# alp-aydin/Raytracing-Project

Measured on AMD Instinct MI355X. Metric: Mrays/s (primary+secondary) + wall-clock per frame, 4K scene @1/2/4/8 GPU, higher is better.
Workload: dtype f64; 1 GPU; snorlax 3840x2160, 5 lights, rec 4 (config 4); width=3840, height=2160, mode=standard, rays_per_frame=385232714, rays_traced_per_frame=385232714, parallelism=1 ranks, 1 GPU each: row-strips8x1, cull=True

## Files before the change

raytracing-project_amd/csrc/device/rt_device.hpp:

```cpp
#include <hip/hip_runtime.h>
#include <stdint.h>

#include <type_traits>

#include "rt.h"
#include "rt_launch.hpp"
#include "scene_compile.hpp"

#ifndef RT_REAL
#define RT_REAL double
#define RT_NS rtd
#endif

namespace RT_NS {

using rtamd::DevObj;
using rtamd::DevOp;
using real = RT_REAL;
using NodeT = rtamd::NodeR<real>;
using MatT = rtamd::MatR<real>;
using LightT = rtamd::LightR<real>;
using DLightT = rtamd::DLightR<real>;
using FoldT = rtamd::FoldLeafR<real>;
#define RT_STR2(x) #x
// ... 52 lines not shown
    const double rcp = __builtin_amdgcn_rcp(s0);
    const double f0 = __builtin_fma(-s0, rcp, 1.0);
    const double f1 = __builtin_fma(rcp, f0, rcp);
    const double f2 = __builtin_fma(-s0, f1, 1.0);
    const double f3 = __builtin_fma(f1, f2, f1);
    auto quot = [&](double a) {
        bool vcc;
        const double n = __builtin_amdgcn_div_scale(a, b, true, &vcc);
        const double mul = n * f3;
        const double f4 = __builtin_fma(-s0, mul, n);
        return __builtin_amdgcn_div_fixup(__builtin_amdgcn_div_fmas(f4, f3, mul, vcc), b, a);
    };
    return D3{quot(a0), quot(a1), quot(a2)};
}
__device__ __forceinline__ auto div3(float a0, float a1, float a2, float b) {
    struct F3 { float x, y, z; };
    return F3{a0 / b, a1 / b, a2 / b};
}

#ifndef RT_FUSED_NORM
#define RT_FUSED_NORM 1
#endif
static_assert(!RT_FUSED_NORM || std::is_same_v<real, double>, "RT_FUSED_NORM is FP64 only (rt_kernels_f32.hip sets it to 0)");

__device__ __forceinline__ double sqrt_core(double s, double& h) {
    const double y = __builtin_amdgcn_rsq(s);
    double g = s * y;
    h = y * 0.5;
    const double r = __builtin_fma(-h, g, 0.5);
    g = __builtin_fma(g, r, g);
    h = __builtin_fma(h, r, h);
    const double d0 = __builtin_fma(-g, g, s);
    g = __builtin_fma(d0, h, g);
    const double d1 = __builtin_fma(-g, g, s);
    return __builtin_fma(d1, h, g);
}

__device__ __forceinline__ D3 div3(double a0, double a1, double a2, double L, double h) {
    const double y0 = h + h;
    const double e = __builtin_fma(-L, y0, 1.0);
    const double y = __builtin_fma(y0, e, y0);
    auto quot = [&](double a) {
        const double q = a * y;
        const double r = __builtin_fma(-L, q, a);
        return __builtin_fma(r, y, q);
    };
// ... 82 lines not shown
    PH_CHAIN_XF,
    PH_OBJ_PREF,
    PH_OBJ_HIT,
    PH_WAVE_SETUP,
    PH_COUNT
};
enum RtEvent {
    EV_SHQ = 0,
    EV_SH_CAND,
    EV_SH_HIT,
    EV_SH_CSG,
    EV_PR_CAND,
    EV_PR_HIT,
    EV_FOLD_LEAF,
    EV_COMB,
    EV_COMB_SINGLE,
    EV_COMB_EASY,
    EV_COMB_GEN,
    EV_LIGHT1,
    EV_LIGHT2,
    EV_BOUNCE,
    EV_COMPACT_LEAF,
    EV_WAVES,
    EV_COUNT
};
template <bool C>
struct Cnt;
template <>
struct Cnt<false> {
    static constexpr bool kPlain = false;
    __device__ __forceinline__ void inc(int) {}
    __device__ __forceinline__ void gate(bool) {}
#ifdef RT_EVENT_PROF
    __device__ static unsigned long long* acc() {
        __shared__ unsigned long long a[4][EV_COUNT];
        return &a[threadIdx.x >> 6][0];
    }
    __device__ __forceinline__ void init() {
        if ((threadIdx.x & 63) == 0)
            for (int k = 0; k < EV_COUNT; ++k) acc()[k] = 0;
    }
    __device__ __forceinline__ bool first() {
        return (int)__lane_id() == __builtin_ctzll(__builtin_amdgcn_read_exec());
    }
    __device__ __forceinline__ void ev(int k) {
        if (first()) acc()[k] += 1;
    }
// ... 579 lines not shown
        real t1 = (-half_b + s) / RV(1.0);
        if (t0 > t1) {
            const real tt = t0;
            t0 = t1;
            t1 = tt;
        }
        o.t0 = t0;
        o.t1 = t1;
        if (o.ok) cnt.inc(RT_OPC_SPHERE_IVL_HIT);
    }
    o.s0 = o.t0;
    o.s1 = o.t1;
}

template <class CT>
__device__ __forceinline__ void csg_c(int op, const CIvl& A, const CIvl& B, CIvl& R, CT& cnt) {
    R.ok = 0;
    R.t0 = R.t1 = R.s0 = R.s1 = RV(0.0);
    R.c0 = R.c1 = 0;
    if (!A.ok && !B.ok) return;
    cnt.inc(RT_OPC_CSG_COMBINE);
    cnt.ev(EV_COMB);
    if (!(A.ok && B.ok)) {
        cnt.ev(EV_COMB_SINGLE);
        const bool useA = A.ok;
        if (op == RT_CSG_INTERSECTION || (op == RT_CSG_DIFFERENCE && !useA)) return;
        const CIvl& X = useA ? A : B;
        const bool inX = (X.t0 < RV(1e-6)) && (X.t1 > RV(1e-6));
        R.t1 = X.t1;
        R.s1 = X.s1;
        R.c1 = X.c1;
        if (inX) {
            R.ok = __builtin_isfinite(X.t1);
            R.t0 = RV(0.0);
            R.s0 = X.s0;
            R.c0 = (X.c0 & ~REF_FLIP) | REF_ORIGIN;
        } else {
            R.ok = __builtin_isfinite(X.t0) && __builtin_isfinite(X.t1) && !ev_less(X.t1, 1, X.t0, 0);
            R.t0 = X.t0;
            R.s0 = X.s0;
            R.c0 = X.c0;
        }
        return;
    }
    if (op == RT_CSG_UNION) {
        const real e = RV(1e-6);
        const bool easy = __builtin_isfinite(A.t0) && __builtin_isfinite(A.t1) && __builtin_isfinite(B.t0) &&
                          __builtin_isfinite(B.t1) && (A.t1 - A.t0 > e) && (B.t1 - B.t0 > e) &&
                          (fabs_r(A.t0 - B.t0) > e) && (fabs_r(A.t0 - B.t1) > e) && (fabs_r(A.t1 - B.t0) > e) &&
                          (fabs_r(A.t1 - B.t1) > e);
        if (easy) {
            cnt.ev(EV_COMB_EASY);
            const bool inA = (A.t0 < e) && (A.t1 > e);
            const bool inB = (B.t0 < e) && (B.t1 > e);
            const bool xa = inA || (!inB && A.t0 < B.t0);
            const real x1 = xa ? A.t1 : B.t1;
            const real y0 = xa ? B.t0 : A.t0;
            const real y1 = xa ? B.t1 : A.t1;
            const bool ext_y = (y0 < x1) && (y1 > x1);
            const bool org = inA || inB;
            const int xc0 = xa ? A.c0 : B.c0;
            R.ok = 1;
            R.t0 = org ? RV(0.0) : (xa ? A.t0 : B.t0);
            R.s0 = xa ? A.s0 : B.s0;
            R.c0 = org ? ((xc0 & ~REF_FLIP) | REF_ORIGIN) : xc0;
            R.t1 = ext_y ? y1 : x1;
            R.s1 = (ext_y != xa) ? A.s1 : B.s1;
            R.c1 = (ext_y != xa) ? A.c1 : B.c1;
            return;
        }
    }
    cnt.ev(EV_COMB_GEN);
    real et[4];
    int ec[4];
#pragma unroll
    for (int k = 0; k < 4; ++k) {
        et[k] = RV(0.0);
        ec[k] = 0;
    }
    int n = 0;
    {
        const real tv[4] = {A.t0, A.t1, B.t0, B.t1};
        const bool pv[4] = {A.ok && __builtin_isfinite(A.t0), A.ok && __builtin_isfinite(A.t1),
                            B.ok && __builtin_isfinite(B.t0), B.ok && __builtin_isfinite(B.t1)};
#pragma unroll
        for (int e = 0; e < 4; ++e) {
#pragma unroll
            for (int k = 0; k < 4; ++k) {
                const bool here = pv[e] && n == k;
                et[k] = here ? tv[e] : et[k];
                ec[k] = here ? e : ec[k];
            }
            n += pv[e] ? 1 : 0;
        }
    }
// ... 560 lines not shown
    const f2v qxy = pk_fma(f2s(-s), K.uxy, wxy);
    const float qz = __builtin_fmaf(-s, K.uz, wz);
    const float d2 = dot_pk(qxy, qz, qxy, qz);
    const float R = g.w + K.rho + __builtin_fmaf(1e-5f, gmag, K.m5);
    return !(d2 > R * R);
}
__device__ __forceinline__ bool capsule_touch(const float* g, const Capsule& K) {
    const float4 b = *reinterpret_cast<const float4*>(g);
    return capsule_touch(b, ball_mag(b), K);
}


__device__ __forceinline__ bool record_touch(const float4 c0, const float4 c1, const Capsule& K) {
    const int type = __float_as_int(c1.x);
    const f2v sab = pk_fma(f2s(c0.x), K.abx, pk_fma(f2s(c0.y), K.aby, f2s(c0.z) * K.abz)) - f2s(c0.w);
    const float m = __builtin_fmaf(1e-5f, c1.y, K.rm5);
    const bool plane = !((sab.x > m) & (sab.y > m)) & !((sab.x < -m) & (sab.y < -m));
    const bool ball = capsule_touch(c0, c1.y, K);
    return (type == 1) | ((type == 2) & ball) | ((type == 3) & plane);
}

template <bool EAGER, bool DEEP, bool UO, bool BV = false, bool LEAD = false, class CT>
__device__ bool scene_occluded_capsule(const DevScene& S, const DRay& r0, real tmin, real tmax, bool need, bool wave_ok,
                                    CT& cnt, bool regular = true) {
#if defined(RT_ABL) && RT_ABL == 1
    return false;
#endif
    cnt.pb(PH_WAVE_SETUP);
    const FRay fr = to_fray(r0);
    DRay r = r0;
    bool r_exact = false;
    const float ftmin = (float)tmin, ftmax = (float)tmax;
    const uint64_t nm = __ballot(need);
    if (!nm) return false;
    cnt.ev(EV_SHQ);
    const int f = __builtin_ctzll(nm);
    const float Ax = __builtin_fmaf(ftmin, fr.dx, fr.ox), Ay = __builtin_fmaf(ftmin, fr.dy, fr.oy),
                Az = __builtin_fmaf(ftmin, fr.dz, fr.oz);
    const float Bx = __builtin_fmaf(ftmax, fr.dx, fr.ox), By = __builtin_fmaf(ftmax, fr.dy, fr.oy),
                Bz = __builtin_fmaf(ftmax, fr.dz, fr.oz);
    const bool fin = __builtin_isfinite(Ax + Ay + Az + Bx + By + Bz) && regular;
    const bool cap = wave_ok && exec_full() && !__any(need && !fin);
    const float ax = rdlane_f(Ax, f), ay = rdlane_f(Ay, f), az = rdlane_f(Az, f);
    const float bx = rdlane_f(Bx, f), by = rdlane_f(By, f), bz = rdlane_f(Bz, f);
    const float da = (Ax - ax) * (Ax - ax) + (Ay - ay) * (Ay - ay) + (Az - az) * (Az - az);
    const float db = (Bx - bx) * (Bx - bx) + (By - by) * (By - by) + (Bz - bz) * (Bz - bz);
    const float d = need ? __builtin_fmaxf(da, db) : 0.0f;
// ... 52 lines not shown
        const int nc = S.n_objs - base;
        const int j = base + lane;
        const int jr = j < S.n_objs ? j : S.n_objs - 1;
        const float4 c0 = S.ctab[2 * jr], c1 = S.ctab[2 * jr + 1];
        const bool pass = (j < S.n_objs) &
                          (cap ? record_touch(c0, c1, K)
                               : __float_as_int(c1.x) != 0);
        m = (cap && exec_full()) ? __ballot(pass) : (nc >= 64 ? ~0ull : ((1ull << nc) - 1));
        cnt.pe(PH_WAVE_SETUP);
#if defined(RT_ABL) && RT_ABL == 2
        if (m != 12345) return false;
#endif
        if constexpr (kCounting<CT>) {
            if (need) {
                int skipped = 0;
                for (int o = base; o < S.n_objs && o < base + 64; ++o) {
                    const int k = S.objs[o].kind;
                    if (k != rtamd::OBJ_GROUP && k != rtamd::OBJ_NEVER && !((m >> (o - base)) & 1)) ++skipped;
                }
                cnt_add(cnt, RT_OPC_CULLED, skipped);
            }
        }
        }
        while (m) {
            const int o = base + __builtin_ctzll(m);
            m &= m - 1;
            const DevObj ob = S.objs[o];
            if (ob.kind == rtamd::OBJ_GROUP || ob.kind == rtamd::OBJ_NEVER) continue;
            cnt.ev(EV_SH_CAND);
            cnt.pb(PH_OBJ_PREF);
            uint64_t lmask = ~0ull;
            bool use_mask = false;
            if (kCsg<CT> && cap && ob.npb > 0 && exec_full()) {
                const float* g = S.gb + 4 * (ob.pb0 + (lane < ob.npb ? lane : 0));
                const bool in = lane < ob.npb;
                const uint64_t cb = __ballot(in && capsule_touch(g, K));
                bool seg = cb != 0;
#ifndef RT_NO_LANE_LEAF_TEST
                if (seg) {
                    seg = false;
                    for (uint64_t mm = cb; mm && !seg; mm &= mm - 1) {
                        const float* gk = S.gb + 4 * (ob.pb0 + __builtin_ctzll(mm));
                        seg = __any(need && !hit && ball_touch(gk, fr, ftmin, ftmax));
                    }
                }
#endif
                if (!seg) {
                    if (need) cnt.inc(RT_OPC_CULLED);
                    cnt.pe(PH_OBJ_PREF);
                    continue;
                }
                if (!lb_ready) {
                    lb_ready = true;
// ... 396 lines not shown
            }
            cnt.pe(PH_OBJ_HIT);
            if (csg_obj) cnt.pe(PH_SHADOW_CSG);
            if (__all(hit || !need)) return hit;
        }
    }
    return hit;
}


__device__ __forceinline__ bool cone_touch(const float4 g, float gmag, const Cone& K) {
    return cone_touch_t<false>(g, gmag, K);
}
__device__ __forceinline__ bool cone_touch(const float* g, const Cone& K) {
    const float4 b = *reinterpret_cast<const float4*>(g);
    return cone_touch_t<false>(b, ball_mag(b), K);
}

#ifndef RT_CAM_RHO0
#define RT_CAM_RHO0 1
#endif
template <bool EAGER, bool DEEP, bool BV = false, bool LEAD = false, bool CAM = false, class CT>
__device__ bool scene_intersect_wave(const DevScene& S, const DRay& r, real tmin, real tmax, real& t_best,
                                     DHit& best, bool wave_ok, CT& cnt, bool valid = true) {
    cnt.pb(PH_WAVE_SETUP);
    const uint64_t vm = __ballot(valid);
    if (!vm) {
        cnt.pe(PH_WAVE_SETUP);
        return false;
    }
    const int f = __builtin_ctzll(vm);
    const FRay fr = to_fray(r);
    const bool fin = __builtin_isfinite(fr.ox + fr.oy + fr.oz + fr.dx + fr.dy + fr.dz);
    const bool cone = S.cull && wave_ok && exec_full() && !__any(valid && !fin) && tmin >= RV(0.0);
    const float ox = rdlane_f(fr.ox, f), oy = rdlane_f(fr.oy, f), oz = rdlane_f(fr.oz, f);
    const float ax = rdlane_f(fr.dx, f), ay = rdlane_f(fr.dy, f), az = rdlane_f(fr.dz, f);
    const float dc = valid ? __builtin_fmaxf(0.0f, 1.0f - __builtin_fmaf(fr.dx, ax, __builtin_fmaf(fr.dy, ay, fr.dz * az)))
                           : 0.0f;
    float rho = 0.0f;
    if constexpr (!(CAM && RT_CAM_RHO0)) {
        const float do2 = valid ? (fr.ox - ox) * (fr.ox - ox) + (fr.oy - oy) * (fr.oy - oy) + (fr.oz - oz) * (fr.oz - oz)
                                : 0.0f;
        rho = cone ? sqrt_cull(__uint_as_float(wave_max_u32(__float_as_uint(do2)))) : 0.0f;
    }
    const float dcm = cone ? __uint_as_float(wave_max_u32(__float_as_uint(dc))) + 4e-6f : 2.0f;
    const float cth = 1.0f - dcm;
    const bool wide = !(cth > 0.0f);
    const float sth = sqrt_cull(__builtin_fmaxf(0.0f, 1.0f - cth * cth)) + 1e-6f;
// ... 109 lines not shown
                                         (t == closest && (win < 0 ? tie : (oo > win_orig ? tie : !win_tie))));
                if (take) {
                    closest = t;
                    win = o;
                    win_orig = oo;
                    win_tie = tie;
                    wp = p;
                    wts = ts;
                    wcode = code;
                }
            } else if (object_hit<EAGER, DEEP>(S, ob, r, tmin, closest, t, p, ts, code, cnt, lmask, use_mask)) {
                closest = t;
                win = o;
                wp = p;
                wts = ts;
                wcode = code;
            }
            cnt.gate(true);
            cnt.pe(PH_OBJ_HIT);
            if (csg_obj) cnt.pe(PH_PRIMARY_CSG);
        }
    }
    if (win < 0) return false;
    cnt.gate(valid);
    resolve_hit<EAGER>(S, win, r, tmin, wp, wts, wcode, best, cnt);
    cnt.gate(true);
    t_best = closest;
    return true;
}

__device__ __attribute__((noinline)) double pow_general(double x, double y) { return pow(x, y); }
#ifndef RT_POW_ANY_X
#define RT_POW_ANY_X 0
#endif

__device__ __forceinline__ double pow_spec(double x, double y) {
    const int k = (int)y;
    if (!(y >= 0.0 && y < 1024.0 && (double)k == y && (!RT_POW_ANY_X || __builtin_fabs(x) <= 2.0)))
        return pow_general(x, y);
    if (k == 0) return 1.0;
    const int top = 31 - __builtin_clz(k);
    double h = x, l = 0.0;
    for (int i = top - 1; i >= 0; --i) {
        double p = h * h;
        l = __builtin_fma(h + h, l, __builtin_fma(h, h, -p));
        h = p;
// ... 8 lines not shown
__device__ __forceinline__ float pow_spec(float x, float y) { return pow(x, y); }

#ifndef RT_LIGHT_CACHE
#define RT_LIGHT_CACHE 5
#endif
constexpr int kLightCache = RT_LIGHT_CACHE;
constexpr int kPoolWave = (kLightCache > 0 ? kLightCache : 1) * 4 * 64;
constexpr size_t pool_bytes(int threads) { return (size_t)(threads / 64) * kPoolWave * sizeof(double); }
__device__ __forceinline__ double* lds_pool() {
    extern __shared__ double rt_lds_pool[];
    return rt_lds_pool;
}
__device__ __forceinline__ double* wave_pool(int w) { return lds_pool() + (size_t)w * kPoolWave; }

__device__ __forceinline__ V3 combine(V3 a, V3 b) {
    return v3(RV(1.0) - (RV(1.0) - a.x) * (RV(1.0) - b.x), RV(1.0) - (RV(1.0) - a.y) * (RV(1.0) - b.y), RV(1.0) - (RV(1.0) - a.z) * (RV(1.0) - b.z));
}

#ifndef RT_STD_UO
#define RT_STD_UO false
#endif
template <bool EAGER, bool DEEP, bool DL, int WV, bool UO = RT_STD_UO, bool LEAD = false, class CT>
__device__ V3 shade(const DevScene& S, real ht, const DHit& hit, V3 wo, uint32_t& n_occl, CT& cnt,
                    bool valid = true) {
    const bool has_mat = hit.mat >= 0;
    valid = valid && has_mat;
    if (valid) cnt.inc(RT_OPC_SHADE_CALL);
    const bool wave_full = WV && __builtin_amdgcn_read_exec() == ~0ull;
    const V3 n = hit.n;
    const real eps = cmax(RV(1e-3), RV(1e-4) * ht);
    ShadowHull hull{0.0f, 0.0f, 0.0f, 0.0f, 0.0f, false};
    if constexpr (WV == 2) hull = shadow_hull<UO>(hit.p, eps, valid, wave_full);
    V3 E = v3(RV(0.0), RV(0.0), RV(0.0));
    {
        const MatT* m = &S.mats[valid ? hit.mat : 0];
        E = v3(m->ambient[0], m->ambient[1], m->ambient[2]);
    }
    for (int li = 0; DL && li < S.n_dlights; ++li) {
        if (!valid) break;
        const DLightT* L = &S.dlights[li];
        cnt.inc(RT_OPC_LIGHT_EVAL);
        const V3 wi = normalized(v3(-L->dir[0], -L->dir[1], -L->dir[2]));
        const real ndotl = dmax(RV(0.0), dot3(n, wi));
        if (ndotl <= RV(0.0)) continue;
        const V3 so = v3(hit.p.x + n.x * eps, hit.p.y + n.y * eps, hit.p.z + n.z * eps);
        ++n_occl;
        if (scene_occluded<EAGER, DEEP>(S, make_ray(so, wi), eps, RT_INF, cnt)) continue;
        cnt.inc(RT_OPC_SHADE_LIGHT);
        const MatT* m = &S.mats[hit.mat];
        const real sd = m->kd * ndotl;
        const V3 Ed = v3(m->albedo[0] * L->radiance[0] * sd, m->albedo[1] * L->radiance[1] * sd,
                         m->albedo[2] * L->radiance[2] * sd);
        V3 Es = v3(RV(0.0), RV(0.0), RV(0.0));
        if (m->ks > RV(0.0)) {
            cnt.inc(RT_OPC_SHADE_SPEC);
            const V3 rr = normalized(v3(RV(2.0) * dot3(n, wi) * n.x - wi.x, RV(2.0) * dot3(n, wi) * n.y - wi.y,
                                        RV(2.0) * dot3(n, wi) * n.z - wi.z));
            const real rdotv = dmax(RV(0.0), dot3(rr, wo));
            const real spec = pow_spec(rdotv, m->shininess) * m->ks;
            Es = v3(L->radiance[0] * spec, L->radiance[1] * spec, L->radiance[2] * spec);
        }
        E = combine(E, combine(Ed, Es));
    }
    if (WV) cnt.pb(PH_SHADE2);
    double* const lc = wave_pool((int)(threadIdx.x >> 6)) + (threadIdx.x & 63);
    for (int l0 = 0; __any(valid) && l0 < S.n_lights; l0 += 32) {
        const int l1 = S.n_lights - l0 < 32 ? S.n_lights : l0 + 32;
        uint32_t lit = 0;
        if (WV) cnt.pb(PH_SHADE1);
        for (int li = l0; li < l1; ++li) {
            const LightT* L = &S.lights[li];
            if (valid) cnt.inc(RT_OPC_LIGHT_EVAL);
            V3 tl = v3(L->pos[0] - hit.p.x, L->pos[1] - hit.p.y, L->pos[2] - hit.p.z);
            real d2 = dot3(tl, tl);
            const bool clamped = d2 <= RV(0.01);
            if (clamped) d2 = RV(0.01);
#if RT_FUSED_NORM
            const N3 dw = sqrt_div3(tl.x, tl.y, tl.z, d2, valid);
            const real dist = dw.L;
            const auto wq = dw.q;
#else
            const real dist = sqrt_r(d2);
            const auto wq = div3(tl.x, tl.y, tl.z, dist);
#endif
            const V3 wi = v3(wq.x, wq.y, wq.z);
            if (li - l0 < kLightCache) {
                double* c = lc + (li - l0) * 4 * 64;
                c[0] = wi.x;
                c[64] = wi.y;
                c[2 * 64] = wi.z;
                c[3 * 64] = dist;
            }
            const real ndotl = cmax(RV(0.0), dot3(n, wi));
            const real max_t = dist - eps;
            const bool need = valid && ndotl > RV(0.0) && max_t > eps;
            if (!__any(need)) continue;
            cnt.ev(EV_LIGHT1);
            const V3 so = v3(hit.p.x + n.x * eps, hit.p.y + n.y * eps, hit.p.z + n.z * eps);
            bool occ = false;
            if constexpr (WV == 2) {
                cnt.pb(PH_SHADOW);
                occ = scene_occluded_wave<EAGER, DEEP, UO, true>(S, DRay{so, wi}, eps, max_t, need, wave_full, cnt, li,
                                                                 hull, !clamped);
                cnt.pe(PH_SHADOW);
            } else if constexpr (WV) {
                cnt.pb(PH_SHADOW);
                occ = scene_occluded_capsule<EAGER, DEEP, UO, false, LEAD>(S, DRay{so, wi}, eps, max_t, need, wave_full, cnt,
                                                                           !clamped);
                cnt.pe(PH_SHADOW);
            } else if (need) {
                occ = scene_occluded<EAGER, DEEP>(S, DRay{so, wi}, eps, max_t, cnt, true, !clamped);
            }
            if (need) {
                ++n_occl;
                if (!occ) lit |= 1u << (li - l0);
            }
        }
        if (WV) {
            cnt.pe(PH_SHADE1);
            cnt.pb(PH_SHADE2);
        }
#if defined(RT_ABL) && RT_ABL == 4
        if (lit != 12345u) continue;
#endif
        if (!lit) continue;
        const MatT* m = &S.mats[hit.mat];
        const real kd = m->kd, ks = m->ks, shin = m->shininess;
        const V3 alb = ld3(m->albedo);
        for (int li = l0; li < l1; ++li) {
            if (!((lit >> (li - l0)) & 1u)) continue;
            cnt.ev(EV_LIGHT2);
// ... 79 lines not shown
    bool alive = true;
    const bool wave_ok = __builtin_amdgcn_read_exec() == ~0ull;
    auto step = [&](auto first_tag) __attribute__((always_inline)) {
        constexpr bool FIRST = decltype(first_tag)::value;
        const bool eval = alive && depth < limit;
        DRay r;
        if constexpr (FIRST) {
            r = r0;
        } else {
            r = DRay{v3(RV(0.0), RV(0.0), RV(0.0)), v3(RV(0.0), RV(0.0), -RV(1.0))};
            if (eval) r = nxt[rsel];
        }
        if (!FIRST) {
            cnt.ev(EV_BOUNCE);
            cnt.evn(EV_COMPACT_LEAF, (unsigned)__builtin_popcountll(__ballot(eval)));
        }
        real ht = RV(0.0);
        DHit h;
        h.p = h.n = v3(RV(0.0), RV(0.0), RV(0.0));
        h.mat = -1;
        h.ff = 1;
        if (eval) ++n_isect;
        cnt.pb(PH_PRIMARY);
        const bool hit = scene_intersect_wave<EAGER, DEEP, (WV == 2), kCsg<CT> ? RT_SEC_LEAD_I : RT_PLAIN_SEC_LEAD>(S, r, RV(1e-4), RT_INF, ht, h, wave_ok, cnt, eval);
        cnt.pe(PH_PRIMARY);
        const bool sh = eval && hit;
        bool descend = false;
        if (sh && h.mat >= 0) {
            const MatT* mat = &S.mats[h.mat];
            const bool can = depth < limit - 1;
            const bool want_refl = mat->kr > RV(0.0) && can;
            bool want_refr = false;
            DRay refr;
            if (mat->kt > RV(0.0) && can) {
                const real eta = h.ff ? (S.medium_index / mat->refractive_index)
                                      : (mat->refractive_index / S.medium_index);
                const V3 inc = normalized(r.d);
                const real cos_i = -dot3(inc, h.n);
                const real st2 = eta * eta * dmax(RV(0.0), RV(1.0) - cos_i * cos_i);
                if (!(st2 >= RV(1.0))) {
                    want_refr = true;
                    const real cos_t = sqrt_r(RV(1.0) - st2);
                    const real k = eta * cos_i - cos_t;
                    const V3 rd = normalized(v3(inc.x * eta + h.n.x * k, inc.y * eta + h.n.y * k,
                                                inc.z * eta + h.n.z * k));
                    const V3 ro = h.ff ? v3(h.p.x - h.n.x * RV(1e-6), h.p.y - h.n.y * RV(1e-6), h.p.z - h.n.z * RV(1e-6))
                                       : v3(h.p.x + h.n.x * RV(1e-6), h.p.y + h.n.y * RV(1e-6), h.p.z + h.n.z * RV(1e-6));
// ... 2 lines not shown
            }
            if (want_refl || want_refr) {
                WFrame& fr = stk[sp];
                fr.mat = h.mat;
                if (want_refr) nxt[2 * sp + 1] = refr;
                cnt.inc(RT_OPC_SECONDARY);
                if (want_refl) {
                    const V3 inc = normalized(r.d);
                    const real k = RV(2.0) * dot3(inc, h.n);
                    const V3 rd = normalized(v3(inc.x - h.n.x * k, inc.y - h.n.y * k, inc.z - h.n.z * k));
                    const V3 ro = h.ff ? v3(h.p.x + h.n.x * RV(1e-6), h.p.y + h.n.y * RV(1e-6), h.p.z + h.n.z * RV(1e-6))
                                       : v3(h.p.x - h.n.x * RV(1e-6), h.p.y - h.n.y * RV(1e-6), h.p.z - h.n.z * RV(1e-6));
                    fr.sf = want_refr ? 2 : 0;
                    nxt[2 * sp] = make_ray(ro, rd);
                } else {
                    fr.sf = 1;
                }
                ++sp;
                descend = true;
            }
        }
        const V3 wo = normalized(vneg(r.d));
        V3 direct = v3(RV(0.0), RV(0.0), RV(0.0));
        if (__any(sh)) direct = shade<EAGER, DEEP, DL, WV, RT_STD_UO, kCsg<CT> ? RT_SEC_LEAD_S : RT_PLAIN_SEC_LEAD>(S, ht, h, wo, n_occl, cnt, sh);
        V3 ret = v3(RV(0.0), RV(0.0), RV(0.0));
        if (eval && !hit) ret = background(S);
        if (sh) {
            if (descend) {
                stk[sp - 1].total = direct;
                rsel = 2 * (sp - 1) + (stk[sp - 1].sf & 1);
                depth = sp;
            } else {
                ret = direct;
            }
        }
        if (alive && !descend) {
            bool resumed = false;
            while (sp > 0) {
                WFrame& fr = stk[sp - 1];
                const MatT* mat = &S.mats[fr.mat];
                const int sf = fr.sf;
                if ((sf & 1) == 0) {
                    fr.total = combine(fr.total, v3(ret.x * mat->kr, ret.y * mat->kr, ret.z * mat->kr));
                    if (sf & 2) {
                        cnt.inc(RT_OPC_SECONDARY);
                        fr.sf = sf | 1;
                        rsel = 2 * (sp - 1) + 1;
// ... 15 lines not shown
            }
        }
        return ret;
    };
    const V3 first = step(std::true_type{});
    if (!__any(alive)) return first;
    while (__any(alive)) step(std::false_type{});
    return stk[0].total;
}

template <bool EAGER, bool DEEP, bool SECONDARY, bool DL, int WV, class CT>
__device__ __forceinline__ V3 trace(const DevScene& S, DRay r, uint32_t& n_isect, uint32_t& n_occl, CT& cnt) {
#ifndef RT_OLD_TRACE
    if constexpr (SECONDARY && WV) return trace_wave<EAGER, DEEP, DL, WV>(S, r, n_isect, n_occl, cnt);
#endif
    if constexpr (!SECONDARY) {
        if (S.rec_limit <= 0) return v3(RV(0.0), RV(0.0), RV(0.0));
        real ht = RV(0.0);
        DHit h;
        h.mat = -1;
        ++n_isect;
        if constexpr (WV) {
            cnt.pb(PH_PRIMARY);
            const bool hit = scene_intersect_wave<EAGER, DEEP, (WV == 2), false, true>(S, r, RV(1e-4), RT_INF, ht, h,
                                                               __builtin_amdgcn_read_exec() == ~0ull, cnt);
            cnt.pe(PH_PRIMARY);
            if (!__any(hit)) return background(S);
#if defined(RT_ABL) && RT_ABL == 5
            if (S.n_objs != 12345) return hit ? h.n : background(S);
#endif
            const V3 E = shade<EAGER, DEEP, DL, WV>(S, ht, h, normalized(vneg(r.d)), n_occl, cnt, hit);
            return hit ? E : background(S);
        } else {
            if (!scene_intersect<EAGER, DEEP>(S, r, RV(1e-4), RT_INF, ht, h, cnt)) return background(S);
            return shade<EAGER, DEEP, DL, WV>(S, ht, h, normalized(vneg(r.d)), n_occl, cnt);
        }
    }
    Frame stk[kMaxDepth];
    int sp = 0;
    int depth = 0;
    const int limit = S.rec_limit;
    V3 ret;
    for (;;) {
        bool descend = false;
        if (depth >= limit) {
            ret = v3(RV(0.0), RV(0.0), RV(0.0));
        } else {
            real ht = RV(0.0);
            DHit h;
            ++n_isect;
            if (!scene_intersect<EAGER, DEEP>(S, r, RV(1e-4), RT_INF, ht, h, cnt)) {
                ret = background(S);
            } else {
                const V3 wo = normalized(vneg(r.d));
// ... 141 lines not shown
```

raytracing-project_amd/csrc/device/rt_kernels.hpp:

```cpp

namespace RT_NS {

using rtamd::kCounterSlots;
using rtamd::kCounterWords;
using rtamd::PaperParams;
using rtamd::SceneView;
using rtamd::StdParams;

namespace {

#ifndef RT_STD_WPB
#define RT_STD_WPB 1
#endif
constexpr int kStdWPB = RT_STD_WPB;
constexpr int kStdThreads = 64 * kStdWPB;
#ifndef RT_STD_TW
#define RT_STD_TW 2
#endif
constexpr int kStdTW = RT_STD_TW, kStdTH = 8 / RT_STD_TW;
static_assert(kStdTW * kStdTH == 8, "a wave holds 8 pixels");
constexpr int kStdBlockX = kStdWPB >= 2 ? 2 * kStdTW : kStdTW;
constexpr int kStdBlockY = kStdWPB >= 4 ? 2 * kStdTH : kStdTH;

template <bool C, int NWAVES = 4>
// ... 189 lines not shown
#ifndef RT_PAPER_LEAD_S
#define RT_PAPER_LEAD_S true
#endif
template <bool E, bool D, bool C, bool DL = true, int WV = 0, bool T = false, bool PL = false>
__device__ __forceinline__ void paper_primary_body(const DevScene& S, const PaperParams& P) {
    static_assert(!(PL && C), "plain kernels do not count");
    const int lane = threadIdx.x & 63;
    const int x = paper_tile_x() * 8 + (lane & 7);
    const int li = paper_tile_y() * 8 + (lane >> 3);
    const int ei = li < P.n_list ? P.ext_list[li] : -1;
    const bool active = x < P.W && ei >= 0;
    unsigned t_start = 0u;
    if constexpr (T) t_start = (unsigned)wall_clock64();
    uint32_t ni = 0, no = 0;
    std::conditional_t<PL, CntPlain, Cnt<C>> cnt;
    cnt.init();
    DRay r{v3(RV(0.0), RV(0.0), RV(0.0)), v3(RV(0.0), RV(0.0), -RV(1.0))};
    real ht = RV(0.0);
    DHit h;
    h.mat = -1;
    h.p = h.n = v3(RV(0.0), RV(0.0), RV(0.0));
    h.ff = 1;
    bool hits = false, sh = false;
    size_t idx = 0;
    if (active) {
        const int y = P.ext_rows[ei];
        r = gen_ray(S, x, y);
        ++ni;
        if constexpr (WV)
            hits = scene_intersect_wave<E, D, (WV == 2), RT_PAPER_LEAD_I>(S, r, RV(1e-4), RT_INF, ht, h, __builtin_amdgcn_read_exec() == ~0ull,
                                              cnt);
        else
            hits = scene_intersect<E, D>(S, r, RV(1e-4), RT_INF, ht, h, cnt);
        idx = (size_t)ei * P.W + x;
        sh = P.ext_shade[ei] != 0;
    }
    int band = 0;
    if (__any(sh)) {
        V3 base = shade<E, D, DL, WV, PL ? RT_PLAIN_PAPER_UO : RT_PAPER_UO, RT_PAPER_LEAD_S>(S, ht, h, normalized(vneg(r.d)), no,
                                                                                     cnt, sh && hits);
        if (sh) {
            if (!hits) base = v3(RV(1.0), RV(1.0), RV(1.0));
            band = hatch_band(RV(0.299) * base.x + RV(0.587) * base.y + RV(0.114) * base.z);
        }
    }
    if (active) {
        P.t[idx] = ht;
        P.nx[idx] = h.n.x;
        P.ny[idx] = h.n.y;
        P.nz[idx] = h.n.z;
        P.mat[idx] = paper_mat_pack(hits ? h.mat : kPaperMiss, band);
    }
    flush_counters<C, kPaperWPB>(P.counters, ni, no, cnt);
    if constexpr (T) {
        if (__lane_id() == 0) {
            unsigned* slot = paper_wave_slot(P);
            slot[0] = t_start;
            slot[1] = (unsigned)wall_clock64();
        }
    }
}

template <bool E, bool D, bool C, bool T = false>
// ... 330 lines not shown
```

raytracing-project_amd/csrc/device/rt_test_hooks.hip:

```cpp
#include <hip/hip_runtime.h>

#include <algorithm>
#include <atomic>
#include <cstdio>
#include <cstring>
#include <mutex>
#include <string>
#include <vector>

#include "frame_plan.hpp"
#include "jitter_cache.hpp"
#include "mt_jump.hpp"
#include "mt_poly.hpp"
#include "rt.h"
#include "rt_devbuf.hpp"
#include "rt_internal.hpp"
#include "rt_launch.hpp"
#include "rt_test.h"
#include "scene_compile.hpp"

namespace {
using DBuf = rtamd::DevBufT<8>;

int scene_variant(const rt_scene* s, int mode, int flags, rtamd::KernelVariant* v) {
// ... 311 lines not shown
extern "C" int rt_test_compile_forms(const rt_scene* s, int32_t* out, int cap) {
    if (!s || !out || cap < RT_TEST_FORMS_LEN) return RT_ERR_INVALID_ARG;
    try {
        const rtamd::CompiledScene cs = rtamd::compile_scene(*rt_scene_get_desc(s));
        std::fill(out, out + RT_TEST_FORMS_LEN, 0);
        auto bin3 = [](int v) { return v < 0 ? 0 : v > 2 ? 2 : v; };
        for (const auto& o : cs.objs) {
            if (o.kind >= 0 && o.kind <= rtamd::OBJ_GROUP) ++out[RT_TEST_FORMS_OBJ + o.kind];
            if (o.kind != rtamd::OBJ_GROUP && o.has_bound) ++out[RT_TEST_FORMS_BOUNDED];
            if (o.kind != rtamd::OBJ_CHAIN) continue;
            if (o.npb > 0) ++out[RT_TEST_FORMS_PREFILTER];
            ++out[RT_TEST_FORMS_CHAIN_CORE + (o.core ? 1 : 0)];
            ++out[RT_TEST_FORMS_CHAIN_M + std::min(o.m, 3)];
            if (o.m >= 3) ++out[RT_TEST_FORMS_CHAIN_M3_CORE + (o.core ? 1 : 0)];
            if (o.nfold > 0) ++out[RT_TEST_FORMS_FOLD + bin3(o.fold_op)];
        }
        for (const auto& op : cs.ops) {
            if (op.op >= 0 && op.op <= rtamd::OP_IVL_GROUP) ++out[RT_TEST_FORMS_OP + op.op];
            if (op.op == rtamd::OP_NEVER) ++out[RT_TEST_FORMS_NEVER_TOP + bin3(op.top)];
            if (op.op == rtamd::OP_IVL_GROUP) ++out[RT_TEST_FORMS_IVL_GROUP + bin3(op.csg_op)];
        }
        out[RT_TEST_FORMS_RAY_DEPTH] = cs.max_ray_depth;
        out[RT_TEST_FORMS_IVL_DEPTH] = cs.max_ivl_depth;
        return RT_OK;
    } catch (const std::exception& e) {
        rtamd::set_last_error(std::string("scene compile: ") + e.what());
        return RT_ERR_INVALID_ARG;
    }
}

extern "C" int rt_test_plan_dist(int H, int world, int rank, int mode, int kind, int chunks, int32_t* counts,
                                 int32_t* rows_out, int32_t* bounds_out, int32_t* rowtab_out, int cap_table) {
    if (H <= 0 || world <= 0 || rank < 0 || rank >= world || chunks < 1 || chunks > rtamd::kChunks || !counts ||
        !rows_out || !bounds_out)
        return RT_ERR_INVALID_ARG;
    const rtamd::DistPlan p =
        rtamd::plan_dist_frame(H, world, rank, mode, kind ? 0 : rtamd::root_shed(mode), chunks, rowtab_out != nullptr);
    if (rowtab_out && (size_t)cap_table < p.rowtab.size()) return RT_ERR_INVALID_ARG;
    counts[0] = (int32_t)p.rows.size();
    counts[1] = p.m;
    counts[2] = (int32_t)p.bounds.size();
    std::copy(p.rows.begin(), p.rows.end(), rows_out);
    for (size_t k = 0; k < p.bounds.size(); ++k) {
        bounds_out[2 * k] = p.bounds[k].first;
        bounds_out[2 * k + 1] = p.bounds[k].second;
    }
// ... 91 lines not shown
```

raytracing-project_amd/csrc/host/scene_compile.cpp:

```cpp
#include "scene_compile.hpp"

#include <algorithm>
#include <cmath>
#include <cstdlib>
#include <cstring>
#include <stdexcept>

namespace rtamd {
namespace {

struct Bound {
    enum Kind { Empty, Unbounded, Ball } kind = Unbounded;
    double c[3] = {0, 0, 0};
    double r = 0;
    double aniso = 1;
};

Bound ball(double x, double y, double z, double r) {
    Bound b;
    b.kind = Bound::Ball;
    b.c[0] = x; b.c[1] = y; b.c[2] = z;
    b.r = std::fabs(r);
    return b;
}
// ... 409 lines not shown
        }
        cs.max_ray_depth = max_r_;
        cs.max_ivl_depth = max_i_;
        cs.objs = insert_groups(cs.objs);
        cs.ctab.assign(cs.objs.size() * 8, 0.0f);
        for (size_t j = 0; j < cs.objs.size(); ++j) {
            const DevObj& o = cs.objs[j];
            float* c = &cs.ctab[8 * j];
            int type = 1;
            if (o.kind == OBJ_GROUP || o.kind == OBJ_NEVER) {
                type = 0;
            } else if (o.has_bound) {
                type = 2;
                for (int k = 0; k < 4; ++k) c[k] = o.fb[k];
                c[5] = float_ball_mag(c);
            } else if (o.kind == OBJ_HALF) {
                type = 3;
                const double* v = d_.nodes[o.node].v;
                for (int k = 0; k < 3; ++k) c[k] = (float)v[3 + k];
                c[3] = (float)(v[3] * v[0] + v[4] * v[1] + v[5] * v[2]);
                c[5] = (float)(std::fabs(v[0]) + std::fabs(v[1]) + std::fabs(v[2]));
            }
            std::memcpy(&c[4], &type, sizeof(int));
        }
        {
            auto type_of = [&](size_t j) {
                int t;
                std::memcpy(&t, &cs.ctab[8 * j + 4], sizeof t);
                return t;
            };
            size_t lead = 0;
            while (lead < cs.objs.size() && (type_of(lead) == 1 || type_of(lead) == 3)) ++lead;
            bool ok = lead <= 64;
            for (size_t j = lead; ok && j < cs.objs.size(); ++j) ok = type_of(j) != 1 && type_of(j) != 3;
            cs.n_lead = ok ? (int)lead : 0;
        }
        build_wave_bvh(cs);
        light_records(cs.ctab.data(), cs.objs.size(), 8, d_.lights, d_.n_lights, cs.lrec);
        light_records(cs.wctab.data(), cs.wobjs.size(), 8, d_.lights, d_.n_lights, cs.lwrec);
        light_records(cs.gbounds.data(), cs.gbounds.size() / 4, 4, d_.lights, d_.n_lights, cs.lgb);
        return cs;
    }

    static void build_wave_bvh(CompiledScene& cs) {
        std::vector<int> ids;
        for (size_t j = 0; j < cs.objs.size(); ++j)
// ... 141 lines not shown
    int64_t i;
    std::memcpy(&i, &x, sizeof i);
    return i >= 0 ? i : -(i & INT64_MAX);
}
double dval(int64_t k) {
    const int64_t i = k >= 0 ? k : ((-k) | INT64_MIN);
    double x;
    std::memcpy(&x, &i, sizeof x);
    return x;
}
template <class P>
double least_true(P pred) {
    int64_t lo = dkey(-1.0), hi = dkey(1.0);
    if (!pred(dval(hi))) return 2.0;
    if (pred(dval(lo))) return -1.0;
    while (hi - lo > 1) {
        const int64_t mid = lo + (hi - lo) / 2;
        (pred(dval(mid)) ? hi : lo) = mid;
    }
    return dval(hi);
}
}

void pokeball_thresholds(double btn_outer, double ring_width, double& xb, double& xi) {
    const double inner = std::max(0.0, btn_outer - ring_width);
    xb = least_true([&](double x) { return std::acos(x) <= btn_outer; });
    const double lt = least_true([&](double x) { return std::acos(x) < inner; });
    xi = lt == 2.0 ? 1.0 : lt == -1.0 ? -2.0 : dval(dkey(lt) - 1);
}

CompiledScene compile_scene(const rt_scene_desc& d) {
    Compiler c(d);
    return c.run();
}

}

extern "C" int rt_test_pokeball_thresholds(double btn_outer, double ring_width, double* out2) {
    if (!out2) return -1;
    rtamd::pokeball_thresholds(btn_outer, ring_width, out2[0], out2[1]);
    return 0;
}
```

raytracing-project_amd/csrc/host/scene_compile.hpp:

```cpp
#pragma once

#include <cstdint>
#include <string>
#include <vector>

#include "rt.h"

namespace rtamd {

enum DevObjKind : int32_t {
    OBJ_SPHERE = 0,
    OBJ_HALF = 1,
    OBJ_POKE = 2,
    OBJ_CHAIN = 3,
    OBJ_EAGER = 4,
    OBJ_NEVER = 5,
    OBJ_GROUP = 6
};

enum DevOpCode : int32_t {
    OP_XPUSH = 0,
    OP_LEAF_IVL = 1,
    OP_CSG = 2,
    OP_XPOP_IVL = 3,
// ... 49 lines not shown
    std::vector<int32_t> worig;
    std::vector<float> wchunk;
    std::vector<float> lrec, lwrec, lgb;
    int max_ray_depth = 0;
    int max_ivl_depth = 0;
    bool has_eager = false;
    int n_lead = 0;
    bool has_pokeball = false;
};

constexpr int kWaveChunk = 64;
constexpr int kWaveBvhMin = 4 * kWaveChunk;

#ifdef __HIP__
__host__ __device__
#endif
inline bool accepts_tie(const DevObj& o) {
    return o.kind == OBJ_SPHERE || o.kind == OBJ_HALF || o.kind == OBJ_POKE ||
           (o.kind == OBJ_CHAIN && o.m == 0 && o.core == 0);
}

CompiledScene compile_scene(const rt_scene_desc& d);

constexpr int kPokeXb = 20, kPokeXi = 21;
void pokeball_thresholds(double btn_outer, double ring_width, double& xb, double& xi);

}
```

raytracing-project_amd/python/rtamd.py:

```python
from __future__ import annotations

import ctypes as C
import os
from dataclasses import dataclass

import numpy as np

_HERE = os.path.dirname(os.path.abspath(__file__))
PKG_DIR = os.path.dirname(_HERE)
REPO_DIR = os.path.dirname(PKG_DIR)
LIB_DIR = os.path.join(PKG_DIR, "lib")
BIN_DIR = os.path.join(PKG_DIR, "bin")
ORACLE_DIR = os.path.join(REPO_DIR, "oracle")

RT_OK = 0
RT_MODE_STANDARD = 0
RT_MODE_PAPER = 1
RT_OK = 0
RT_ERR_INVALID_ARG = -1
RT_ERR_HIP = -5
RT_ERR_UNSUPPORTED = -6
RT_ERR_NO_DEVICE = -7
RT_FLAG_NONE = 0
RT_FLAG_COUNT_OPS = 1
# ... 424 lines not shown

OBJ_KINDS = ("sphere", "half", "poke", "chain", "eager", "never", "group")
OP_CODES = ("xpush", "leaf_ivl", "csg", "xpop_ivl", "leaf_isect", "csg_isect", "xpop_hit", "never", "ivl_group")
CSG_OPS = ("union", "intersection", "difference")


def compile_forms(scene: Scene) -> dict:
    lib = amd_lib()
    lib.rt_test_compile_forms.argtypes = [C.c_void_p, C.POINTER(C.c_int32), C.c_int]
    n = 37
    out = (C.c_int32 * n)()
    rc = lib.rt_test_compile_forms(scene.handle, out, n)
    if rc != RT_OK:
        raise RTError(rc, last_error())
    keys = ([f"obj/{k}" for k in OBJ_KINDS] + ["chain_core/leaf", "chain_core/csg"] +
            [f"chain_m/{m}" for m in ("0", "1", "2", "3+")] + ["chain_m3+/leaf", "chain_m3+/csg"] +
            [f"fold/{o}" for o in CSG_OPS] + [f"op/{k}" for k in OP_CODES] +
            [f"never_top/{t}" for t in (0, 1, 2)] + [f"ivl_group/{o}" for o in CSG_OPS] +
            ["max_ray_depth", "max_ivl_depth", "bounded", "prefilter"])
    assert len(keys) == n
    return dict(zip(keys, (int(v) for v in out)))


KERNEL_TABLES = ("rtd std", "rtd paper", "rtf std", "rtf paper", "rtdb std", "rtdb paper", "rtd query", "rtdb query",
                 "finish")


def kernel_rows(table: int) -> list[str]:
    lib = amd_lib()
    lib.rt_test_kernel_row.argtypes = [C.c_int, C.c_int, C.c_char_p, C.c_int]
    buf = C.create_string_buffer(160)
    out = []
    while lib.rt_test_kernel_row(table, len(out), buf, 160) == RT_OK:
        out.append(buf.value.decode())
    return out


def launch_log(on: bool) -> None:
    _ok(amd_lib().rt_test_launch_log(1 if on else 0), "rt_test_launch_log")


def launch_log_get() -> list[str]:
    lib = amd_lib()
    lib.rt_test_launch_log_get.argtypes = [C.c_char_p, C.c_int]
    cap = 1 << 16
    while True:
# ... 749 lines not shown
```

Baseline: 62760 Mrays/s.

## Skip self-occlusion test for the hit object in wave shadow queries

Threads the winning object index from primary intersection into shading. When a whole wave hit the same simple sphere or halfspace leaf, and the shadow origin lies provably outside it with the light on the open side (ndotl above a small tau), the owning object is removed from the shadow candidate mask. This avoids re-testing each ray's own surface in every shadow ray. It costs extra wave ballots, a node lookup, a per-object classification done at scene compile time, and an extra register for the winner index. It also adds an optional capsule-plane cull, off by default, and profiling event aliases.

New measurement: 63010 Mrays/s, median of 6. About the same (+0.4%).

```diff
diff --git a/raytracing-project_amd/csrc/device/rt_device.hpp b/raytracing-project_amd/csrc/device/rt_device.hpp
--- a/raytracing-project_amd/csrc/device/rt_device.hpp
+++ b/raytracing-project_amd/csrc/device/rt_device.hpp
@@ -98,6 +98,20 @@
 #define RT_FUSED_NORM 1
 #endif
 static_assert(!RT_FUSED_NORM || std::is_same_v<real, double>, "RT_FUSED_NORM is FP64 only (rt_kernels_f32.hip sets it to 0)");
+
+#ifndef RT_OWN_LEAF
+#define RT_OWN_LEAF 1
+#endif
+constexpr bool kOwnLeaf = RT_OWN_LEAF && std::is_same_v<real, double>;
+constexpr double kOwnTau = 1.0 / 67108864.0;
+#ifndef RT_CAPSULE_PLANE
+#define RT_CAPSULE_PLANE 0
+#endif
+#if defined(RT_EVENT_PROF) && (RT_EVENT_PROF + 0) == 2
+#define RT_EVENT_OWN 1
+#else
+#define RT_EVENT_OWN 0
+#endif
 
 __device__ __forceinline__ double sqrt_core(double s, double& h) {
     const double y = __builtin_amdgcn_rsq(s);
@@ -226,7 +240,10 @@
     EV_BOUNCE,
     EV_COMPACT_LEAF,
     EV_WAVES,
-    EV_COUNT
+    EV_COUNT,
+    EV_SH_OWN_SPHERE = EV_COMB_SINGLE,
+    EV_SH_OWN_HALF = EV_COMB_EASY,
+    EV_SH_OWN_OTHER = EV_COMB_GEN
 };
 template <bool C>
 struct Cnt;
@@ -852,7 +869,7 @@
     cnt.inc(RT_OPC_CSG_COMBINE);
     cnt.ev(EV_COMB);
     if (!(A.ok && B.ok)) {
-        cnt.ev(EV_COMB_SINGLE);
+        if (!RT_EVENT_OWN) cnt.ev(EV_COMB_SINGLE);
         const bool useA = A.ok;
         if (op == RT_CSG_INTERSECTION || (op == RT_CSG_DIFFERENCE && !useA)) return;
         const CIvl& X = useA ? A : B;
@@ -880,7 +897,7 @@
                           (fabs_r(A.t0 - B.t0) > e) && (fabs_r(A.t0 - B.t1) > e) && (fabs_r(A.t1 - B.t0) > e) &&
                           (fabs_r(A.t1 - B.t1) > e);
         if (easy) {
-            cnt.ev(EV_COMB_EASY);
+            if (!RT_EVENT_OWN) cnt.ev(EV_COMB_EASY);
             const bool inA = (A.t0 < e) && (A.t1 > e);
             const bool inB = (B.t0 < e) && (B.t1 > e);
             const bool xa = inA || (!inB && A.t0 < B.t0);
@@ -900,7 +917,7 @@
             return;
         }
     }
-    cnt.ev(EV_COMB_GEN);
+    if (!RT_EVENT_OWN) cnt.ev(EV_COMB_GEN);
     real et[4];
     int ec[4];
 #pragma unroll
@@ -1507,7 +1524,7 @@
 
 template <bool EAGER, bool DEEP, bool UO, bool BV = false, bool LEAD = false, class CT>
 __device__ bool scene_occluded_capsule(const DevScene& S, const DRay& r0, real tmin, real tmax, bool need, bool wave_ok,
-                                    CT& cnt, bool regular = true) {
+                                    CT& cnt, bool regular = true, int own = -1, bool own_skip = false) {
 #if defined(RT_ABL) && RT_ABL == 1
     return false;
 #endif
@@ -1606,13 +1623,31 @@
             }
         }
         }
+        if constexpr (kOwnLeaf && !BV) {
+            const int b = own - base;
+            if ((RT_EVENT_OWN ? own_skip : own >= 0) && b >= 0 && b < 64 && ((m >> b) & 1ull)) {
+                m &= ~(1ull << b);
+                if (need) cnt.inc(RT_OPC_CULLED);
+            }
+        }
         while (m) {
             const int o = base + __builtin_ctzll(m);
             m &= m - 1;
             const DevObj ob = S.objs[o];
             if (ob.kind == rtamd::OBJ_GROUP || ob.kind == rtamd::OBJ_NEVER) continue;
             cnt.ev(EV_SH_CAND);
+#if RT_EVENT_OWN
+            if (o == own) cnt.ev(ob.kind == rtamd::OBJ_HALF ? EV_SH_OWN_HALF : ob.kind <= rtamd::OBJ_POKE ? EV_SH_OWN_SPHERE : EV_SH_OWN_OTHER);
+#endif
             cnt.pb(PH_OBJ_PREF);
+#if RT_CAPSULE_PLANE
+            if (S.cull && ch >= 0 && ob.kind == rtamd::OBJ_HALF &&
+                !__any(need && !hit && (!regular || plane_touch(S.ctab[2 * o], S.ctab[2 * o + 1], fr, ftmin, ftmax)))) {
+                if (need) cnt.inc(RT_OPC_CULLED);
+                cnt.pe(PH_OBJ_PREF);
+                continue;
+            }
+#endif
             uint64_t lmask = ~0ull;
             bool use_mask = false;
             if (kCsg<CT> && cap && ob.npb > 0 && exec_full()) {
@@ -2055,8 +2090,9 @@
 #endif
 template <bool EAGER, bool DEEP, bool BV = false, bool LEAD = false, bool CAM = false, class CT>
 __device__ bool scene_intersect_wave(const DevScene& S, const DRay& r, real tmin, real tmax, real& t_best,
-                                     DHit& best, bool wave_ok, CT& cnt, bool valid = true) {
+                                     DHit& best, int& win_out, bool wave_ok, CT& cnt, bool valid = true) {
     cnt.pb(PH_WAVE_SETUP);
+    win_out = -1;
     const uint64_t vm = __ballot(valid);
     if (!vm) {
         cnt.pe(PH_WAVE_SETUP);
@@ -2212,6 +2248,7 @@
         }
     }
     if (win < 0) return false;
+    win_out = win;
     cnt.gate(valid);
     resolve_hit<EAGER>(S, win, r, tmin, wp, wts, wcode, best, cnt);
     cnt.gate(true);
@@ -2266,7 +2303,7 @@
 #endif
 template <bool EAGER, bool DEEP, bool DL, int WV, bool UO = RT_STD_UO, bool LEAD = false, class CT>
 __device__ V3 shade(const DevScene& S, real ht, const DHit& hit, V3 wo, uint32_t& n_occl, CT& cnt,
-                    bool valid = true) {
+                    bool valid = true, int own = -1) {
     const bool has_mat = hit.mat >= 0;
     valid = valid && has_mat;
     if (valid) cnt.inc(RT_OPC_SHADE_CALL);
@@ -2306,6 +2343,38 @@
         }
         E = combine(E, combine(Ed, Es));
     }
+    int own_o = -1;
+    int own_u = -1;
+    if constexpr (WV == 1 && (kOwnLeaf || RT_EVENT_OWN)) {
+        const uint64_t vm = __ballot(valid);
+        if (S.cull && vm && exec_full()) {
+            const int o = __builtin_amdgcn_readlane(own, __builtin_ctzll(vm));
+            if (o >= 0 && !__any(valid && own != o)) {
+                own_u = o;
+                if constexpr (kOwnLeaf) {
+                    const float4 c1 = S.ctab[2 * o + 1];
+                    const int el = __float_as_int(c1.z);
+                    if (el != 0) {
+                        const NodeT* nd = &S.nodes[__float_as_int(c1.w)];
+                        const V3 so = v3(hit.p.x + n.x * eps, hit.p.y + n.y * eps, hit.p.z + n.z * eps);
+                        bool pre;
+                        if (el == 1) {
+                            const real rad = nd->v[3];
+                            const V3 oc = v3(so.x - nd->v[0], so.y - nd->v[1], so.z - nd->v[2]);
+                            const real cterm = dot3(oc, oc) - rad * rad;
+                            pre = hit.ff != 0 && cterm >= RV(0.0) && dot3(n, n) <= RV(4.0);
+                        } else {
+                            const V3 ns = ld3(nd->v + 3);
+                            const V3 diff = v3(nd->v[0] - so.x, nd->v[1] - so.y, nd->v[2] - so.z);
+                            const real num = dot3(ns, diff);
+                            pre = hit.ff != 0 ? num <= RV(0.0) : num >= RV(0.0);
+                        }
+                        if (!__any(valid && !pre)) own_o = o;
+                    }
+                }
+            }
+        }
+    }
     if (WV) cnt.pb(PH_SHADE2);
     double* const lc = wave_pool((int)(threadIdx.x >> 6)) + (threadIdx.x & 63);
     for (int l0 = 0; __any(valid) && l0 < S.n_lights; l0 += 32) {
@@ -2349,8 +2418,13 @@
                 cnt.pe(PH_SHADOW);
             } else if constexpr (WV) {
                 cnt.pb(PH_SHADOW);
+                bool own_skip = false;
+                if constexpr (kOwnLeaf) {
+                    if (own_o >= 0)
+                        own_skip = exec_full() && !__any(need && !(!clamped && ndotl >= RV(kOwnTau)));
+                }
                 occ = scene_occluded_capsule<EAGER, DEEP, UO, false, LEAD>(S, DRay{so, wi}, eps, max_t, need, wave_full, cnt,
-                                                                           !clamped);
+                                                                           !clamped, (RT_EVENT_OWN || own_skip) ? (RT_EVENT_OWN ? own_u : own_o) : -1, own_skip);
                 cnt.pe(PH_SHADOW);
             } else if (need) {
                 occ = scene_occluded<EAGER, DEEP>(S, DRay{so, wi}, eps, max_t, cnt, true, !clamped);
@@ -2476,7 +2550,8 @@
         h.ff = 1;
         if (eval) ++n_isect;
         cnt.pb(PH_PRIMARY);
-        const bool hit = scene_intersect_wave<EAGER, DEEP, (WV == 2), kCsg<CT> ? RT_SEC_LEAD_I : RT_PLAIN_SEC_LEAD>(S, r, RV(1e-4), RT_INF, ht, h, wave_ok, cnt, eval);
+        int win = -1;
+        const bool hit = scene_intersect_wave<EAGER, DEEP, (WV == 2), kCsg<CT> ? RT_SEC_LEAD_I : RT_PLAIN_SEC_LEAD>(S, r, RV(1e-4), RT_INF, ht, h, win, wave_ok, cnt, eval);
         cnt.pe(PH_PRIMARY);
         const bool sh = eval && hit;
         bool descend = false;
@@ -2525,7 +2600,7 @@
         }
         const V3 wo = normalized(vneg(r.d));
         V3 direct = v3(RV(0.0), RV(0.0), RV(0.0));
-        if (__any(sh)) direct = shade<EAGER, DEEP, DL, WV, RT_STD_UO, kCsg<CT> ? RT_SEC_LEAD_S : RT_PLAIN_SEC_LEAD>(S, ht, h, wo, n_occl, cnt, sh);
+        if (__any(sh)) direct = shade<EAGER, DEEP, DL, WV, RT_STD_UO, kCsg<CT> ? RT_SEC_LEAD_S : RT_PLAIN_SEC_LEAD>(S, ht, h, wo, n_occl, cnt, sh, win);
         V3 ret = v3(RV(0.0), RV(0.0), RV(0.0));
         if (eval && !hit) ret = background(S);
         if (sh) {
@@ -2587,14 +2662,15 @@
         ++n_isect;
         if constexpr (WV) {
             cnt.pb(PH_PRIMARY);
-            const bool hit = scene_intersect_wave<EAGER, DEEP, (WV == 2), false, true>(S, r, RV(1e-4), RT_INF, ht, h,
+            int win = -1;
+            const bool hit = scene_intersect_wave<EAGER, DEEP, (WV == 2), false, true>(S, r, RV(1e-4), RT_INF, ht, h, win,
                                                                __builtin_amdgcn_read_exec() == ~0ull, cnt);
             cnt.pe(PH_PRIMARY);
             if (!__any(hit)) return background(S);
 #if defined(RT_ABL) && RT_ABL == 5
             if (S.n_objs != 12345) return hit ? h.n : background(S);
 #endif
-            const V3 E = shade<EAGER, DEEP, DL, WV>(S, ht, h, normalized(vneg(r.d)), n_occl, cnt, hit);
+            const V3 E = shade<EAGER, DEEP, DL, WV>(S, ht, h, normalized(vneg(r.d)), n_occl, cnt, hit, win);
             return hit ? E : background(S);
         } else {
             if (!scene_intersect<EAGER, DEEP>(S, r, RV(1e-4), RT_INF, ht, h, cnt)) return background(S);
diff --git a/raytracing-project_amd/csrc/device/rt_kernels.hpp b/raytracing-project_amd/csrc/device/rt_kernels.hpp
--- a/raytracing-project_amd/csrc/device/rt_kernels.hpp
+++ b/raytracing-project_amd/csrc/device/rt_kernels.hpp
@@ -235,13 +235,14 @@
     h.p = h.n = v3(RV(0.0), RV(0.0), RV(0.0));
     h.ff = 1;
     bool hits = false, sh = false;
+    int win = -1;
     size_t idx = 0;
     if (active) {
         const int y = P.ext_rows[ei];
         r = gen_ray(S, x, y);
         ++ni;
         if constexpr (WV)
-            hits = scene_intersect_wave<E, D, (WV == 2), RT_PAPER_LEAD_I>(S, r, RV(1e-4), RT_INF, ht, h, __builtin_amdgcn_read_exec() == ~0ull,
+            hits = scene_intersect_wave<E, D, (WV == 2), RT_PAPER_LEAD_I>(S, r, RV(1e-4), RT_INF, ht, h, win, __builtin_amdgcn_read_exec() == ~0ull,
                                               cnt);
         else
             hits = scene_intersect<E, D>(S, r, RV(1e-4), RT_INF, ht, h, cnt);
@@ -251,7 +252,7 @@
     int band = 0;
     if (__any(sh)) {
         V3 base = shade<E, D, DL, WV, PL ? RT_PLAIN_PAPER_UO : RT_PAPER_UO, RT_PAPER_LEAD_S>(S, ht, h, normalized(vneg(r.d)), no,
-                                                                                     cnt, sh && hits);
+                                                                                     cnt, sh && hits, win);
         if (sh) {
             if (!hits) base = v3(RV(1.0), RV(1.0), RV(1.0));
             band = hatch_band(RV(0.299) * base.x + RV(0.587) * base.y + RV(0.114) * base.z);
diff --git a/raytracing-project_amd/csrc/device/rt_test_hooks.hip b/raytracing-project_amd/csrc/device/rt_test_hooks.hip
--- a/raytracing-project_amd/csrc/device/rt_test_hooks.hip
+++ b/raytracing-project_amd/csrc/device/rt_test_hooks.hip
@@ -357,6 +357,15 @@
         }
         out[RT_TEST_FORMS_RAY_DEPTH] = cs.max_ray_depth;
         out[RT_TEST_FORMS_IVL_DEPTH] = cs.max_ivl_depth;
+        if (cap >= RT_TEST_FORMS_LEN_OWN) {
+            out[RT_TEST_FORMS_OWN_SPHERE] = out[RT_TEST_FORMS_OWN_HALF] = 0;
+            for (size_t j = 0; j < cs.objs.size(); ++j) {
+                int own;
+                std::memcpy(&own, &cs.ctab[8 * j + 6], sizeof own);
+                if (own == 1) ++out[RT_TEST_FORMS_OWN_SPHERE];
+                if (own == 2) ++out[RT_TEST_FORMS_OWN_HALF];
+            }
+        }
         return RT_OK;
     } catch (const std::exception& e) {
         rtamd::set_last_error(std::string("scene compile: ") + e.what());
diff --git a/raytracing-project_amd/csrc/host/scene_compile.cpp b/raytracing-project_amd/csrc/host/scene_compile.cpp
--- a/raytracing-project_amd/csrc/host/scene_compile.cpp
+++ b/raytracing-project_amd/csrc/host/scene_compile.cpp
@@ -455,6 +455,10 @@
                 c[5] = (float)(std::fabs(v[0]) + std::fabs(v[1]) + std::fabs(v[2]));
             }
             std::memcpy(&c[4], &type, sizeof(int));
+            const int own = o.kind <= OBJ_POKE ? own_leaf_class(d_.nodes[o.node]) : 0;
+            const int node = own ? o.node : 0;
+            std::memcpy(&c[6], &own, sizeof(int));
+            std::memcpy(&c[7], &node, sizeof(int));
         }
         {
             auto type_of = [&](size_t j) {
@@ -642,6 +646,20 @@
 }
 }
 
+int own_leaf_class(const rt_node& leaf) {
+    const double* v = leaf.v;
+    if (leaf.kind == RT_NODE_SPHERE || leaf.kind == RT_NODE_POKEBALL) {
+        const double l1 = std::fabs(v[0]) + std::fabs(v[1]) + std::fabs(v[2]);
+        return (std::isfinite(v[3]) && v[3] > 0.0 && l1 <= kOwnLeafMaxOffset * v[3]) ? 1 : 0;
+    }
+    if (leaf.kind == RT_NODE_HALFSPACE) {
+        const double len = std::sqrt(v[3] * v[3] + v[4] * v[4] + v[5] * v[5]);
+        const bool fin = std::isfinite(v[0]) && std::isfinite(v[1]) && std::isfinite(v[2]);
+        return (fin && std::fabs(len - 1.0) <= 1e-9) ? 2 : 0;
+    }
+    return 0;
+}
+
 void pokeball_thresholds(double btn_outer, double ring_width, double& xb, double& xi) {
     const double inner = std::max(0.0, btn_outer - ring_width);
     xb = least_true([&](double x) { return std::acos(x) <= btn_outer; });
diff --git a/raytracing-project_amd/csrc/host/scene_compile.hpp b/raytracing-project_amd/csrc/host/scene_compile.hpp
--- a/raytracing-project_amd/csrc/host/scene_compile.hpp
+++ b/raytracing-project_amd/csrc/host/scene_compile.hpp
@@ -95,6 +95,9 @@
 
 CompiledScene compile_scene(const rt_scene_desc& d);
 
+constexpr double kOwnLeafMaxOffset = 256.0;
+int own_leaf_class(const rt_node& leaf);
+
 constexpr int kPokeXb = 20, kPokeXi = 21;
 void pokeball_thresholds(double btn_outer, double ring_width, double& xb, double& xi);
 
diff --git a/raytracing-project_amd/python/rtamd.py b/raytracing-project_amd/python/rtamd.py
--- a/raytracing-project_amd/python/rtamd.py
+++ b/raytracing-project_amd/python/rtamd.py
@@ -470,6 +470,17 @@
     return dict(zip(keys, (int(v) for v in out)))
 
 
+def own_leaf_forms(scene: Scene) -> dict:
+    lib = amd_lib()
+    lib.rt_test_compile_forms.argtypes = [C.c_void_p, C.POINTER(C.c_int32), C.c_int]
+    n = 39
+    out = (C.c_int32 * n)()
+    rc = lib.rt_test_compile_forms(scene.handle, out, n)
+    if rc != RT_OK:
+        raise RTError(rc, last_error())
+    return {"own/sphere": int(out[37]), "own/half": int(out[38])}
+
+
 KERNEL_TABLES = ("rtd std", "rtd paper", "rtf std", "rtf paper", "rtdb std", "rtdb paper", "rtd query", "rtdb query",
                  "finish")
 
```
